# ebartrum/lightning_gan_zoo

Hardware: AMD Instinct MI355X
Metric: images/sec (G+D step) at 64x64 bs=128/GPU (higher is better)
Workload: dtype f32; 1 GPU; dc_gan synthetic 64x64 bs=128/GPU, one optimizer cycle of 2 batches (Lightning alternation + toggle), reference optimizer, fp32; key=dc_gan_bs128, global_batch=128, parallelism=dp1, images_counted=2*bs*n_gpus per step (every batch of the cycle)

## Files before the change

include/gz_ops.h:

```cpp
#ifndef GZ_OPS_H
#define GZ_OPS_H

#include <stddef.h>

#ifdef __cplusplus
extern "C" {
#endif

#ifndef __HIP__
typedef struct ihipStream_t* hipStream_t;
#endif

#define GZ_ACT_NONE 0
#define GZ_ACT_RELU 1
#define GZ_ACT_LRELU 2
#define GZ_ACT_TANH 3


long long gz_conv2d_pack_fwd_elems(int K, int C, int KH, int KW);
long long gz_conv2d_pack_dgrad_elems(int K, int C, int KH, int KW, int S);

int gz_conv2d_pack_fwd(const float* w, float* wpack, int K, int C, int KH, int KW, hipStream_t stream);
int gz_conv2d_pack_dgrad(const float* w, float* wpack, int K, int C, int KH, int KW, int S, int P,
                         hipStream_t stream);
// ... 104 lines not shown
                      int PH, int PW, int act, float slope, hipStream_t stream);
int gz_conv2d_fwd_any_into(const float* x, const float* wpack, const float* bias, float* y, int y_image_channels, int N,
                           int C, int H, int W, int K, int OH, int OW, int KH, int KW, int SH, int SW, int PH, int PW,
                           int act, float slope, hipStream_t stream);
int gz_pool2d(const float* x, float* y, long long planes, int H, int W, int OH, int OW, int KS, int S, int P, int mode,
              hipStream_t stream);
int gz_resize_bilinear(const float* x, float* y, long long planes, int H, int W, int OH, int OW, float mul, float add,
                       hipStream_t stream);

int gz_bce_logits_mean(const float* x, float* loss, int n, float target, hipStream_t stream);
int gz_bce_logits_mean_bwd(const float* x, const float* gloss, float* dx, int n, float target, hipStream_t stream);
int gz_pair_loss(const float* x, float* loss, int n_each, float t0, float t1, int mode, hipStream_t stream);
int gz_pair_loss_bwd(const float* x, const float* gloss, float* dx, int n_each, float t0, float t1, int mode,
                     hipStream_t stream);
int gz_gp_penalty(const float* sumsq, float* out, int n, hipStream_t stream);
int gz_gp_penalty_bwd(const float* sumsq, const float* gout, float* dsumsq, int n, hipStream_t stream);
int gz_mse_mean(const float* a, const float* b, float* loss, int n, hipStream_t stream);
int gz_mse_mean_bwd(const float* a, const float* b, const float* gloss, float* da, int n, hipStream_t stream);
int gz_vec_normalize(const float* x, float* out, float* out2, float* norm_out, int n, float eps, hipStream_t stream);
int gz_vec_normalize_dot(const float* x, float* out, float* out2, float* dot_out, int n, float eps,
                         hipStream_t stream);
int gz_vec_dot(const float* a, const float* b, float* out, int n, hipStream_t stream);
int gz_sn_max_jobs(void);
size_t gz_sn_table_bytes(void);
long long gz_sn_workspace_floats(int R, int L);
int gz_sn_add(void* table_host, const float* W, float* u, float* v, float* us, float* vs, float* sigma, float* workspace,
              int R, int L);
int gz_sn_power_iteration(void* table_host, float eps, hipStream_t stream);
int gz_sn_sigma_coef_floats(int groups);
int gz_sn_sigma_term(const float* rowsums, const float* rstd, const float* sigma, const float* u, const float* v,
                     float* coefs, float* term, int rows, int groups, int R, int L, float eps, hipStream_t stream);
int gz_div_scalar(const float* x, const float* sigma, float* out, long long count, hipStream_t stream);
int gz_spectral_norm_bwd(const float* g, const float* rowdots, const float* u, const float* v, const float* sigma,
                         float* out, int R, int L, hipStream_t stream);

size_t gz_norm_workspace_bytes(int N, int C);
int gz_norm_coef_elems(int N, int C, int per_channel);

int gz_batchnorm_finalize(const float* partials, int rows, long long count, const float* gamma, const float* beta,
                          float* coef, float* running_mean, float* running_var, long long* num_batches_tracked, int C,
                          float eps, float momentum, hipStream_t stream);
int gz_batchnorm_stats(const float* x, const float* gamma, const float* beta, float* coef, float* running_mean,
                       float* running_var, long long* num_batches_tracked, void* workspace, int N, int C,
                       int inner, float eps, float momentum, hipStream_t stream);
int gz_channel_sum(const float* x, float* out, void* workspace, int N, int C, int inner, hipStream_t stream);
int gz_batchnorm_eval_coef(const float* gamma, const float* beta, const float* running_mean,
                           const float* running_var, float* coef, int C, float eps, hipStream_t stream);
int gz_rownorm_stats(const float* x, const float* gamma, const float* beta, float* coef, void* workspace, int N,
                     int C, int inner, float eps, int affine_per_row, int unbiased, hipStream_t stream);
int gz_rownorm_act_fwd(const float* x, const float* gamma, const float* beta, float* coef, float* out, int N, int C,
                       int inner, float eps, int affine_per_row, int unbiased, int act, float slope,
                       hipStream_t stream);
int gz_adain_const_fwd(const float* x, const float* sb, float* coef, float* out, int N, int C, int inner, float eps,
                       int act, float slope, hipStream_t stream);
int gz_adain_const_bwd(const float* gout, const float* x, const float* coef, float* dx, float* dsb, int N, int C,
                       int inner, int act, float slope, hipStream_t stream);
int gz_norm_act_fwd(const float* x, const float* coef, float* out, int N, int C, int inner, int per_channel,
                    int act, float slope, hipStream_t stream);
int gz_rownorm_act_fwd_sigma(const float* x, const float* sigma, int groups, float* coef, float* out, int N, int C,
                             int inner, float eps, int act, float slope, hipStream_t stream);
int gz_rownorm_act_bwd_rows(const float* gout, const float* x, const float* coef, float* dx, float* rowsums, int N, int C,
                            int inner, int act, float slope, hipStream_t stream);
int gz_norm_act_bwd(const float* gout, const float* x, const float* coef, float* dx, float* dgamma, float* dbeta,
                    void* workspace, float* kbuf, int N, int C, int inner, int per_channel, int affine_per_row,
                    int unbiased, int act, float slope, hipStream_t stream);
int gz_batchnorm_stats_g(const float* x, const float* gamma, const float* beta, float* coef, float* running_mean,
                         float* running_var, long long* num_batches_tracked, void* workspace, int N, int C,
                         int inner, float eps, float momentum, int groups, hipStream_t stream);
int gz_batchnorm_finalize_g(const float* partials, int rows, long long count, const float* gamma, const float* beta,
                            float* coef, float* running_mean, float* running_var, long long* num_batches_tracked,
                            int C, float eps, float momentum, int groups, hipStream_t stream);
int gz_batchnorm_act_fwd_fused(const float* x, const float* partials, int rows, long long count, const float* gamma,
                               const float* beta, float* coef, float* running_mean, float* running_var,
                               long long* num_batches_tracked, void* workspace, float* out, int N, int C, int inner,
                               float eps, float momentum, int groups, int act, float slope, hipStream_t stream);
int gz_norm_act_fwd_g(const float* x, const float* coef, float* out, int N, int C, int inner, int per_channel,
                      int groups, int act, float slope, hipStream_t stream);
int gz_rownorm_act_bwd_acc(const float* gout, const float* x, const float* coef, float* dx, float* dgamma, float* dbeta,
                           void* workspace, float* kbuf, int N, int C, int inner, int act, float slope, int accumulate,
                           hipStream_t stream);
int gz_batchnorm_act_bwd_g(const float* gout, const float* x, const float* coef, float* dx, float* dgamma, float* dbeta,
                           void* workspace, float* kbuf, int N, int C, int inner, int act, float slope, int groups,
                           int accumulate, hipStream_t stream);

int gz_rownorm_act_bwd2(const float* gout, const float* v, const float* x, const float* coef, float* gg_out,
                        float* gx, float* ggamma, void* workspace, int N, int C, int inner, int act, float slope,
                        hipStream_t stream);
int gz_act_bwd(const float* g, const float* out, float* dx, long long count, int act, float slope,
               hipStream_t stream);
int gz_tanh_bwd2(const float* v, const float* g, const float* out, float* res, long long count, hipStream_t stream);

int gz_rowdot(const float* a, const float* b, float* y, int R, int L, int b_broadcast, hipStream_t stream);
int gz_rowscale(const float* x, const float* s, const float* x2, const float* s2, float* out, int R, int L,
                int x_broadcast, int one_minus_s, hipStream_t stream);
int gz_linear_multi_max_jobs(void);
size_t gz_linear_multi_table_bytes(void);
int gz_linear_multi_add(void* table_host, const float* weight, const float* bias, float* out, const float* g, float* dw,
                        float* db, int J);
int gz_linear_multi_fwd(void* table_host, const float* x, int N, int K, int act, float slope, hipStream_t stream);
int gz_linear_multi_bwd(void* table_host, const float* x, int N, int K, int act, float slope, hipStream_t stream);
int gz_colsum(const float* x, float* out, int R, int L, hipStream_t stream);
size_t gz_coldot_workspace_bytes(int R, int L);
int gz_coldot(const float* g, const float* x, float* out, float* workspace, size_t ws_bytes, int R, int L,
              hipStream_t stream);
int gz_coldot_partial(const float* g, const float* x, float* out, float* workspace, size_t ws_bytes, int R, int L,
                      int* nz_out, hipStream_t stream);
int gz_copy_words(const void* src, void* dst, long long words, hipStream_t stream);
int gz_clamp_(float* p, long long count, float lo, float hi, hipStream_t stream);

int gz_act_fwd(const float* x, float* y, long long count, int act, float slope, hipStream_t stream);
int gz_axpby(const float* a, float alpha, const float* b, float beta, float* out, float* act_out, long long count,
             int act, float slope, hipStream_t stream);
int gz_avgpool3s2_fwd(const float* x, float* y, long long planes, int H, int W, int OH, int OW, hipStream_t stream);
int gz_avgpool3s2_bwd(const float* gy, float* gx, long long planes, int H, int W, int OH, int OW,
                      hipStream_t stream);
int gz_upsample2_fwd(const float* x, float* y, long long planes, int H, int W, hipStream_t stream);
int gz_upsample2_bwd(const float* gy, float* gx, long long planes, int H, int W, hipStream_t stream);

int gz_u8hwc_to_nchw(const unsigned char* in, float* out, int N, int H, int W, int C, float mean, float std,
                     hipStream_t stream);

#define GZ_OPT_MAX_TENSORS 24
int gz_adam_step(int count, float* const* params, float* const* grads, float* const* exp_avg,
                 float* const* exp_avg_sq, const long long* numel, float lr, float beta1, float beta2, float eps,
                 int step, float grad_scale, int zero_grads, hipStream_t stream);
int gz_adam_src_max_tensors(void);
size_t gz_adam_src_table_bytes(void);
int gz_adam_src_add(void* table_host, float* param, float* exp_avg, float* exp_avg_sq, long long numel,
                    const float* slabs, int nz, long long stride);
int gz_adam_step_from_slabs(void* table_host, float lr, float beta1, float beta2, float eps, int step, float grad_scale,
                            hipStream_t stream);
int gz_adam_tick(float* tick, float beta1, float beta2, hipStream_t stream);
int gz_adam_step_dev(int count, float* const* params, float* const* grads, float* const* exp_avg,
                     float* const* exp_avg_sq, const long long* numel, float lr, float beta1, float beta2, float eps,
                     const float* tick, float grad_scale, int zero_grads, hipStream_t stream);
int gz_rmsprop_step(int count, float* const* params, float* const* grads, float* const* square_avg,
                    const long long* numel, float lr, float alpha, float eps, float grad_scale, int zero_grads,
                    hipStream_t stream);

const char* gz_last_error(void);

const char* gz_build_info(void);
const char* gz_source_digest(void);

#ifdef __cplusplus
}
#endif
#endif
```

lightning_gan_zoo_amd/csrc/gz_knobs.h:

```cpp
#pragma once
#include <stdlib.h>
#include <string.h>
#include <atomic>

namespace gz {

#define GZ_KNOB_LIST(X)                                                                                               \
                                                                                          \
    X(bool, no_igemm2, "GZ_NO_IGEMM2", false)                        \
    X(bool, no_igemm2_tap, "GZ_NO_IGEMM2_TAP", false)                      \
    X(bool, no_plane_a, "GZ_NO_PLANE_A", false)                \
    X(bool, no_wg3r, "GZ_NO_WG3R", false)                               \
    X(int, wg3r_wgs, "GZ_WG3R_WGS", 2)                              \
    X(int, wg3r_min_chunks, "GZ_WG3R_MIN_CHUNKS", 24)                         \
    X(bool, no_fewk_wg, "GZ_NO_FEWK_WG", false)               \
    X(bool, no_fewk_conv, "GZ_NO_FEWK_CONV", false)            \
    X(int, dg3_tile, "GZ_DG3_TILE", 0)                       \
    X(int, dg3_wgs, "GZ_DG3_WGS", 2)                         \
    X(int, dg3_min_chunks, "GZ_DG3_MIN_CHUNKS", 32)                            \
    X(bool, no_igemm2_wg, "GZ_NO_IGEMM2_WG", false)                              \
    X(bool, no_igemm2w, "GZ_NO_IGEMM2W", false)              \
    X(bool, no_igemm2wg, "GZ_NO_IGEMM2WG", false)                          \
    X(int, igemm2_tile, "GZ_IGEMM2_TILE", 0)                                 \
    X(bool, no_tile64, "GZ_NO_TILE64", false)                                  \
    X(bool, no_kg2, "GZ_NO_KG2", false)                             \
    X(bool, no_pool_plane, "GZ_NO_POOL_PLANE", false)               \
    X(bool, no_pool_group, "GZ_NO_POOL_GROUP", false)                  \
    X(bool, no_any2, "GZ_NO_ANY2", false)                    \
    X(bool, no_dg5, "GZ_NO_DG5", false)                      \
    X(int, dg5_wgs, "GZ_DG5_WGS", 512)                              \
    X(int, dg5_min_chunks, "GZ_DG5_MIN_CHUNKS", 24)             \
    X(int, dg5_min_units, "GZ_DG5_MIN_UNITS", 80)             \
    X(int, kg2_min_chunks, "GZ_KG2_MIN_CHUNKS", 32)                           \
    X(int, tap64_min_chunks, "GZ_TAP64_MIN_CHUNKS", 32)      \
    X(int, tile, "GZ_TILE", -1)                                               \
    X(int, min_wgs, "GZ_MIN_WGS", 0)                                \
    X(bool, no_big_split, "GZ_NO_BIG_SPLIT", false)                                                                   \
    X(bool, no_splitk, "GZ_NO_SPLITK", false)                                                                         \
    X(int, split_target, "GZ_SPLIT_TARGET", 1024)                                                                     \
    X(int, split_below, "GZ_SPLIT_BELOW", 512)                                                                        \
    X(bool, no_tapmajor, "GZ_NO_TAPMAJOR", false)                                                                     \
    X(bool, no_row4, "GZ_NO_ROW4", false)                                                                             \
    X(int, fwd2_min_tiles, "GZ_FWD2_MIN_TILES", 16)                                                                   \
    X(int, dg2_min_tiles, "GZ_DG2_MIN_TILES", 64)                                                                     \
    X(int, tap_wgs, "GZ_TAP_WGS", 384)                                                                                \
    X(int, tap_cps_max, "GZ_TAP_CPS_MAX", 96)                                                                         \
    X(int, wg_target, "GZ_WG_TARGET", 1024)                                                                           \
    X(int, wg2_min_chunks, "GZ_WG2_MIN_CHUNKS", 0)                                                                    \
    X(bool, wg_generic, "GZ_WG_GENERIC", false)                                                                       \
                                                                                                  \
    X(bool, no_smallc, "GZ_NO_SMALLC", false)                                                                         \
    X(bool, no_smallc5, "GZ_NO_SMALLC5", false)                                                                       \
    X(bool, smallc_one_pos, "GZ_SMALLC_ONE_POS", false)                                                               \
    X(long long, smallc_split_below, "GZ_SMALLC_SPLIT_BELOW", 192 * 1024)                                             \
    X(long long, smallc_split8_below, "GZ_SMALLC_SPLIT8_BELOW", 36 * 1024)                                            \
    X(int, smallc_ks, "GZ_SMALLC_KS", 0)                                                                              \
    X(bool, no_fewc_wg, "GZ_NO_FEWC_WG", false)                                                                       \
    X(bool, no_act_fuse, "GZ_NO_ACT_FUSE", false)                                                                     \
    X(bool, no_pack_k4, "GZ_NO_PACK_K4", false)                                                                       \
    X(bool, no_resample_swizzle, "GZ_NO_RESAMPLE_SWIZZLE", false)                                                     \
    X(int, fewc_wg_blocks, "GZ_FEWC_WG_BLOCKS", 512)                                                                  \
    X(bool, no_smallch_conv, "GZ_NO_SMALLCH_CONV", false)                                                             \
    X(bool, no_smallch_wg, "GZ_NO_SMALLCH_WG", false)                                                                 \
    X(int, c3_gpw, "GZ_C3_GPW", 4)                                                                                    \
                                                                                        \
    X(bool, no_xcd_swizzle, "GZ_NO_XCD_SWIZZLE", false)                                                               \
    X(int, dyn_lds, "GZ_DYN_LDS", 0)                                                                                  \
    X(int, igemm2_stagger, "GZ_IGEMM2_STAGGER", 0)                                                                    \
    X(int, igemm2_lds, "GZ_IGEMM2_LDS", 0)                                                                            \
                                                                     \
    X(bool, dg3_even_split, "GZ_DG3_EVEN_SPLIT", false)                                                               \
    X(int, wg3_target, "GZ_WG3_TARGET", 1024)                                                                         \
    X(int, wg3_tile, "GZ_WG3_TILE", -1)                                                                               \
    X(bool, norm_unfused, "GZ_NORM_UNFUSED", false)                                                                   \
    X(int, norm_bwd_cache, "GZ_NORM_BWD_CACHE", 4)                                                                    \
    X(bool, resample_fwd_direct, "GZ_RESAMPLE_FWD_DIRECT", false)                                                     \
    X(int, resample_bwd_mode, "GZ_RESAMPLE_BWD", 0)

struct Knobs {
    bool experiments;
#define GZ_KNOB_FIELD(type, name, env, dflt) type name;
    GZ_KNOB_LIST(GZ_KNOB_FIELD)
#undef GZ_KNOB_FIELD
};

inline void knob_read(bool& v, const char* e) { v = e != nullptr; }
inline void knob_read(int& v, const char* e) {
    if (!e) return;
    if (!strcmp(e, "scatter")) v = 1;
    else if (!strcmp(e, "gather")) v = 2;
    else v = atoi(e);
}
inline void knob_read(long long& v, const char* e) { if (e) v = atoll(e); }

inline const Knobs& knobs() {
    static const Knobs k = [] {
        Knobs n;
#define GZ_KNOB_INIT(type, name, env, dflt) n.name = dflt;
        GZ_KNOB_LIST(GZ_KNOB_INIT)
#undef GZ_KNOB_INIT
        const char* on = getenv("GZ_EXPERIMENTS");
        n.experiments = on && on[0] && on[0] != '0';
        if (n.experiments) {
#define GZ_KNOB_ENV(type, name, env, dflt) knob_read(n.name, getenv(env));
            GZ_KNOB_LIST(GZ_KNOB_ENV)
#undef GZ_KNOB_ENV
        }
        return n;
    }();
    return k;
}

inline std::atomic<int>& cu_budget_ref() {
    static std::atomic<int> v{256};
    return v;
}
inline int cus() { return cu_budget_ref().load(std::memory_order_relaxed); }

}
```

lightning_gan_zoo_amd/csrc/gz_norm.hip:

```cpp
#include "gz_common.h"
#include "gz_knobs.h"
#include "../../include/gz_ops.h"

namespace gz {

constexpr int PW_THREADS = 256;

struct RowGeom {
    int rows, q4;
    int lpr, rpw;
};

static RowGeom row_geom(long long rows, int inner) {
    RowGeom g;
    g.rows = (int)rows;
    g.q4 = inner / 4;
    int lpr = 1;
    while (lpr < 64 && lpr < g.q4) lpr <<= 1;
    g.lpr = lpr;
    g.rpw = 64 / lpr;
    return g;
}

static int row_grid(const RowGeom& g) {
    long long groups = ((long long)g.rows + g.rpw - 1) / g.rpw;
    long long blocks = (groups + 3) / 4;
    if (blocks > 256 * 8) blocks = 256 * 8;
    if (blocks < 1) blocks = 1;
    return (int)blocks;
}

template <int NS>
__device__ __forceinline__ void sub_reduce(float (&s)[NS], int lpr) {
    for (int o = lpr >> 1; o > 0; o >>= 1) {
#pragma unroll
        for (int k = 0; k < NS; ++k) s[k] += __shfl_xor(s[k], o, 64);
    }
}

__global__ __launch_bounds__(PW_THREADS) void row_sums_kernel(const float* __restrict__ x, f32x2* __restrict__ sums,
                                                              RowGeom g) {
    const int lane = threadIdx.x & 63;
    const int wave = (blockIdx.x * PW_THREADS + threadIdx.x) >> 6;
    const int nwaves = (gridDim.x * PW_THREADS) >> 6;
    const int sub = lane / g.lpr, l = lane % g.lpr;
    for (long long row0 = (long long)wave * g.rpw; row0 < g.rows; row0 += (long long)nwaves * g.rpw) {
        long long row = row0 + sub;
        float s[2] = {0.f, 0.f};
        if (row < g.rows) {
            const f32x4* p = reinterpret_cast<const f32x4*>(x) + row * g.q4;
            for (int q = l; q < g.q4; q += g.lpr) {
                f32x4 v = p[q];
                s[0] += (v.x + v.y) + (v.z + v.w);
                s[1] += (v.x * v.x + v.y * v.y) + (v.z * v.z + v.w * v.w);
            }
        }
        sub_reduce<2>(s, g.lpr);
        if (row < g.rows && l == 0) sums[row] = f32x2{s[0], s[1]};
    }
}

__global__ __launch_bounds__(64) void channel_sum_finalize_kernel(const f32x2* __restrict__ sums, float* __restrict__ out,
                                                                  int N, int C) {
    const int c = blockIdx.x, lane = threadIdx.x;
    double s = 0.0;
    for (int n = lane; n < N; n += 64) s += (double)sums[(long long)n * C + c].x;
    s = wave_sum_d(s);
    if (lane == 0) out[c] = (float)s;
}

template <int WAVES>
__global__ __launch_bounds__(64 * WAVES) void bn_finalize_kernel(const f32x2* __restrict__ sums,
                                                         const float* __restrict__ gamma,
                                                         const float* __restrict__ beta, float* __restrict__ coef,
                                                         float* running_mean, float* running_var, long long* nbt,
                                                         int N, int C, int inner, float eps, float momentum,
                                                         double count, int groups) {
    const int c = blockIdx.x, lane = threadIdx.x;
    if (c == 0 && lane == 0 && nbt) *nbt += groups;
    const int Ng = N / groups, NC = groups * C;
    for (int g = 0; g < groups; ++g) {
        double s1 = 0.0, s2 = 0.0;
// ... 32 lines not shown
        coef[NC + ci] = be - (float)mean * scale;
        coef[2 * NC + ci] = (float)mean;
        coef[3 * NC + ci] = rstd;
        if (running_mean) {
            double unbiased = cnt > 1.0 ? var * cnt / (cnt - 1.0) : var;
            running_mean[c] = (1.f - momentum) * running_mean[c] + momentum * (float)mean;
            running_var[c] = (1.f - momentum) * running_var[c] + momentum * (float)unbiased;
        }
    }
}

__global__ void bn_eval_coef_kernel(const float* __restrict__ gamma, const float* __restrict__ beta,
                                    const float* __restrict__ rm, const float* __restrict__ rv,
                                    float* __restrict__ coef, int C, float eps) {
    int c = blockIdx.x * blockDim.x + threadIdx.x;
    if (c >= C) return;
    float rstd = 1.f / sqrtf(rv[c] + eps);
    float ga = gamma ? gamma[c] : 1.f, be = beta ? beta[c] : 0.f;
    coef[c] = ga * rstd;
    coef[C + c] = be - rm[c] * ga * rstd;
    coef[2 * C + c] = rm[c];
    coef[3 * C + c] = rstd;
}

struct ApplyGeom {
    long long total4;
    int q4;
    FastDiv div_q4, div_c;
    int C, per_channel, ncoef;
    int group_rows;
    FastDiv div_grows;
};

__device__ __forceinline__ int coef_index(long long i4, const ApplyGeom& g) {
    uint32_t row = fdiv((uint32_t)i4, g.div_q4);
    if (g.per_channel) {
        const uint32_t grp = g.group_rows ? fdiv(row, g.div_grows) : 0u;
        row = row - fdiv(row, g.div_c) * (uint32_t)g.C + grp * (uint32_t)g.C;
    }
    return (int)row;
}

__global__ __launch_bounds__(PW_THREADS) void norm_act_apply_kernel(const float* __restrict__ x,
                                                                    const float* __restrict__ coef,
                                                                    float* __restrict__ out, ApplyGeom g, int act,
                                                                    float slope) {
    const long long stride = (long long)gridDim.x * PW_THREADS;
    for (long long i = (long long)blockIdx.x * PW_THREADS + threadIdx.x; i < g.total4; i += stride) {
        int ci = coef_index(i, g);
        float sc = coef[ci], sh = coef[g.ncoef + ci];
        f32x4 v = reinterpret_cast<const f32x4*>(x)[i];
        f32x4 o;
#pragma unroll
        for (int k = 0; k < 4; ++k) o[k] = act_fwd(v[k] * sc + sh, act, slope);
        reinterpret_cast<f32x4*>(out)[i] = o;
    }
}

struct BnFuse {
    int N, C, q4, groups, Ng, S, P;
    int CB, run4;
    FastDiv div_q4, div_run;
};

static BnFuse bn_fuse_geom(int N, int C, int inner, int groups) {
    BnFuse f;
    f.N = N; f.C = C; f.q4 = inner / 4; f.groups = groups; f.Ng = N / groups;
    int cb = 1;
    while (cb < 16 && cb * f.q4 < 64 && C % (cb * 2) == 0) cb *= 2;
    f.CB = cb;
    f.run4 = cb * f.q4;
    f.div_q4 = make_fastdiv(f.q4);
    f.div_run = make_fastdiv(f.run4);
    const long long per_cg = (long long)f.Ng * f.run4;
    const long long blocks = (long long)(C / cb) * groups;
    int S = 1;
    while (blocks * S < 1024 && S * 2 <= f.Ng && per_cg / (S * 2) >= 512) S *= 2;
    f.S = S;
    f.P = (f.Ng + S - 1) / S;
    return f;
}

__device__ __forceinline__ void block_channel_sums(const f32x2* __restrict__ base, long long stride, int count, int CB,
                                                   double (*red)[2]) {
    const int tid = threadIdx.x, cb = tid % CB, rr = tid / CB, lanes = PW_THREADS / CB;
    double s1 = 0.0, s2 = 0.0;
    for (int r = rr; r < count; r += lanes) {
        const f32x2 v = base[(long long)r * stride + cb];
        s1 += (double)v.x;
        s2 += (double)v.y;
    }
    __syncthreads();
    red[tid][0] = s1;
    red[tid][1] = s2;
    __syncthreads();
    for (int h = lanes >> 1; h >= 1; h >>= 1) {
        if (rr < h) {
            red[tid][0] += red[tid + h * CB][0];
            red[tid][1] += red[tid + h * CB][1];
        }
        __syncthreads();
    }
}

__global__ __launch_bounds__(PW_THREADS) void bn_apply_fused_kernel(
    const float* __restrict__ x, const f32x2* __restrict__ sums, int rows, double count, const float* __restrict__ gamma,
    const float* __restrict__ beta, float* __restrict__ coef, float* running_mean, float* running_var, long long* nbt,
    float* __restrict__ out, BnFuse f, int inner, float eps, float momentum, int act, float slope) {
    __shared__ double red[PW_THREADS][2];
    __shared__ float mine[16][2];
    const int tid = threadIdx.x;
    const int s = blockIdx.x % f.S, bg = blockIdx.x / f.S, g = bg % f.groups, c0 = (bg / f.groups) * f.CB;
    const bool owner = g == 0 && s == 0;
    const int Rg = rows / f.groups, NC = f.groups * f.C;
    for (int gg = 0; gg < f.groups; ++gg) {
        if (!owner && gg != g) continue;
        block_channel_sums(sums + (long long)gg * Rg * f.C + c0, f.C, Rg, f.CB, red);
        if (tid < f.CB) {
            const int c = c0 + tid;
            const double s1 = red[tid][0], s2 = red[tid][1];
            const double cnt = count > 0.0 ? count : (double)f.Ng * inner;
            const double mean = s1 / cnt;
            double var = s2 / cnt - mean * mean;
            if (var < 0.0) var = 0.0;
            const float rstd = (float)(1.0 / sqrt(var + (double)eps));
            const float ga = gamma ? gamma[c] : 1.f, be = beta ? beta[c] : 0.f;
            const float scale = ga * rstd, shift = be - (float)mean * scale;
            if (gg == g) {
                mine[tid][0] = scale;
                mine[tid][1] = shift;
            }
            if (owner) {
                const int ci = gg * f.C + c;
                coef[ci] = scale;
                coef[NC + ci] = shift;
                coef[2 * NC + ci] = (float)mean;
                coef[3 * NC + ci] = rstd;
                if (running_mean) {
                    const double unbiased = cnt > 1.0 ? var * cnt / (cnt - 1.0) : var;
                    running_mean[c] = (1.f - momentum) * running_mean[c] + momentum * (float)mean;
                    running_var[c] = (1.f - momentum) * running_var[c] + momentum * (float)unbiased;
                }
            }
        }
    }
    if (owner && c0 == 0 && tid == 0 && nbt) *nbt += f.groups;
    __syncthreads();
    const int n0 = g * f.Ng + s * f.P;
    const int n1 = min(g * f.Ng + f.Ng, n0 + f.P);
    const int total = (n1 - n0) * f.run4;
    const f32x4* __restrict__ x4 = reinterpret_cast<const f32x4*>(x);
    f32x4* __restrict__ o4 = reinterpret_cast<f32x4*>(out);
    for (int i = tid; i < total; i += PW_THREADS) {
        const uint32_t p = fdiv((uint32_t)i, f.div_run);
        const uint32_t rem = (uint32_t)i - p * (uint32_t)f.run4;
        const uint32_t cb = fdiv(rem, f.div_q4);
        const long long idx = ((long long)(n0 + (int)p) * f.C + c0) * f.q4 + rem;
        const float sc = mine[cb][0], sh = mine[cb][1];
        const f32x4 v = x4[idx];
        f32x4 o;
#pragma unroll
        for (int k = 0; k < 4; ++k) o[k] = act_fwd(v[k] * sc + sh, act, slope);
        o4[idx] = o;
    }
}

template <int CACHE>
__global__ __launch_bounds__(PW_THREADS) void rownorm_act_fused_kernel(const float* __restrict__ x,
                                                                       const float* __restrict__ gamma,
                                                                       const float* __restrict__ beta,
                                                                       float* __restrict__ coef,
                                                                       float* __restrict__ out, RowGeom g, int C,
                                                                       int inner, float eps, int affine_per_row,
                                                                       int unbiased, int act, float slope,
                                                                       int x_rows, const float* __restrict__ sigma,
                                                                       int sigma_rows) {
    const int lane = threadIdx.x & 63;
// ... 19 lines not shown
                s[0] += (v.x + v.y) + (v.z + v.w);
            }
        }
        sub_reduce<1>(s, g.lpr);
        const double cnt = (double)inner;
        const float mean_f = (float)((double)s[0] / cnt);
        float d[2] = {0.f, 0.f};
        if constexpr (CACHE > 0) {
#pragma unroll
            for (int i = 0; i < CACHE; ++i) {
                if (live && l + i * g.lpr < g.q4) {
#pragma unroll
                    for (int k = 0; k < 4; ++k) {
                        const float e = c[i][k] - mean_f;
                        d[0] += e;
                        d[1] += e * e;
                    }
                }
            }
        } else if (live) {
            for (int q = l; q < g.q4; q += g.lpr) {
                f32x4 v = p[q];
#pragma unroll
                for (int k = 0; k < 4; ++k) {
                    const float e = v[k] - mean_f;
                    d[0] += e;
                    d[1] += e * e;
                }
            }
        }
        sub_reduce<2>(d, g.lpr);
        if (!live) continue;
        const int r = (int)row;
        const double mean = (double)mean_f + (double)d[0] / cnt;
        double var = ((double)d[1] - (double)d[0] * (double)d[0] / cnt) / cnt;
        if (var < 0.0) var = 0.0;
        if (unbiased && inner > 1) var = var * cnt / (cnt - 1.0);
        float eps_r = eps;
        if (sigma) {
            const float sg = sigma[r / sigma_rows];
            eps_r = eps * sg * sg;
        }
        const float rstd = (float)(1.0 / sqrt(var + (double)eps_r));
        const int gi = affine_per_row == 2 ? (r / C) * 2 * C + r % C : (affine_per_row ? r : r % C);
        const float ga = gamma ? gamma[gi] : 1.f, be = beta ? beta[gi] : 0.f;
        const float sc = ga * rstd;
        const float sh = be - (float)mean * sc;
        if (l == 0) {
            coef[r] = sc;
            coef[g.rows + r] = sh;
            coef[2 * g.rows + r] = (float)mean;
            coef[3 * g.rows + r] = rstd;
        }
        if (!out) continue;
        f32x4* po = reinterpret_cast<f32x4*>(out) + row * g.q4;
        if constexpr (CACHE > 0) {
#pragma unroll
            for (int i = 0; i < CACHE; ++i) {
                const int q = l + i * g.lpr;
                if (q < g.q4) {
                    f32x4 o;
#pragma unroll
                    for (int k = 0; k < 4; ++k) o[k] = act_fwd(c[i][k] * sc + sh, act, slope);
                    po[q] = o;
                }
            }
        } else {
            for (int q = l; q < g.q4; q += g.lpr) {
                f32x4 v = p[q], o;
#pragma unroll
                for (int k = 0; k < 4; ++k) o[k] = act_fwd(v[k] * sc + sh, act, slope);
                po[q] = o;
            }
        }
    }
}

__device__ __forceinline__ float act_grad_z(float z, int act, float slope) {
    if (act == ACT_RELU) return z > 0.f ? 1.f : 0.f;
    if (act == ACT_LRELU) return z > 0.f ? 1.f : slope;
    return 1.f;
}

__global__ __launch_bounds__(PW_THREADS) void norm_bwd_rowsums_kernel(const float* __restrict__ gout,
                                                                      const float* __restrict__ x,
                                                                      const float* __restrict__ coef,
                                                                      f32x2* __restrict__ sums, RowGeom g, int C,
                                                                      int per_channel, int ncoef, int act,
                                                                      float slope, int group_rows) {
    const int lane = threadIdx.x & 63;
    const int wave = (blockIdx.x * PW_THREADS + threadIdx.x) >> 6;
    const int nwaves = (gridDim.x * PW_THREADS) >> 6;
    const int sub = lane / g.lpr, l = lane % g.lpr;
    for (long long row0 = (long long)wave * g.rpw; row0 < g.rows; row0 += (long long)nwaves * g.rpw) {
        long long row = row0 + sub;
        float s[2] = {0.f, 0.f};
        if (row < g.rows) {
            int ci = per_channel ? (int)(row % C) + (group_rows ? (int)(row / group_rows) * C : 0) : (int)row;
            float sc = coef[ci], sh = coef[ncoef + ci], mean = coef[2 * ncoef + ci], rstd = coef[3 * ncoef + ci];
            const f32x4* px = reinterpret_cast<const f32x4*>(x) + row * g.q4;
            const f32x4* pg = reinterpret_cast<const f32x4*>(gout) + row * g.q4;
            for (int q = l; q < g.q4; q += g.lpr) {
                f32x4 xv = px[q], gv = pg[q];
#pragma unroll
                for (int k = 0; k < 4; ++k) {
                    float dz = gv[k] * act_grad_z(xv[k] * sc + sh, act, slope);
                    s[0] += dz;
                    s[1] += dz * ((xv[k] - mean) * rstd);
                }
            }
        }
        sub_reduce<2>(s, g.lpr);
        if (row < g.rows && l == 0) sums[row] = f32x2{s[0], s[1]};
    }
}

__global__ __launch_bounds__(64) void bn_bwd_finalize_kernel(const f32x2* __restrict__ sums, float* __restrict__ k,
                                                             float* __restrict__ dgamma, float* __restrict__ dbeta,
                                                             int N, int C, int inner, int groups, int accumulate) {
    const int c = blockIdx.x, lane = threadIdx.x;
    const int Ng = N / groups, NC = groups * C;
    double t1 = 0.0, t2 = 0.0;
    for (int g = 0; g < groups; ++g) {
        double s1 = 0.0, s2 = 0.0;
        for (int n = lane; n < Ng; n += 64) {
            f32x2 v = sums[(long long)(g * Ng + n) * C + c];
            s1 += (double)v.x;
            s2 += (double)v.y;
        }
        s1 = wave_sum_d(s1);
        s2 = wave_sum_d(s2);
        if (lane == 0) {
            double cnt = (double)Ng * inner;
            k[g * C + c] = (float)(s1 / cnt);
            k[NC + g * C + c] = (float)(s2 / cnt);
        }
        t1 += s1;
        t2 += s2;
    }
    if (lane != 0) return;
    if (dgamma) dgamma[c] = (accumulate ? dgamma[c] : 0.f) + (float)t2;
    if (dbeta) dbeta[c] = (accumulate ? dbeta[c] : 0.f) + (float)t1;
}

__global__ void row_bwd_finalize_kernel(const f32x2* __restrict__ sums, float* __restrict__ k,
                                        float* __restrict__ dgamma, float* __restrict__ dbeta, int N, int C,
                                        int inner, int affine_per_row, int unbiased) {
    int i = blockIdx.x * blockDim.x + threadIdx.x;
    int rows = N * C;
    if (i < rows) {
        f32x2 v = sums[i];
        k[i] = v.x / (float)inner;
        k[rows + i] = v.y / (float)((unbiased && inner > 1) ? inner - 1 : inner);
        if (affine_per_row) {
            const int gi = affine_per_row == 2 ? (i / C) * 2 * C + i % C : i;
            if (dgamma) dgamma[gi] = v.y;
            if (dbeta) dbeta[gi] = v.x;
        }
    }
}

__global__ __launch_bounds__(64) void row_bwd_affine_kernel(const f32x2* __restrict__ sums,
                                                            float* __restrict__ dgamma, float* __restrict__ dbeta,
                                                            int N, int C, int accumulate = 0) {
    const int c = blockIdx.x, lane = threadIdx.x;
    double s1 = 0.0, s2 = 0.0;
    for (int n = lane; n < N; n += 64) {
        f32x2 v = sums[(long long)n * C + c];
        s1 += (double)v.x;
        s2 += (double)v.y;
    }
    s1 = wave_sum_d(s1);
    s2 = wave_sum_d(s2);
    if (lane != 0) return;
    if (dgamma) dgamma[c] = (accumulate ? dgamma[c] : 0.f) + (float)s2;
    if (dbeta) dbeta[c] = (accumulate ? dbeta[c] : 0.f) + (float)s1;
}

__global__ __launch_bounds__(PW_THREADS) void norm_bwd_apply_kernel(const float* __restrict__ gout,
                                                                    const float* __restrict__ x,
                                                                    const float* __restrict__ coef,
                                                                    const float* __restrict__ k,
                                                                    float* __restrict__ dx, ApplyGeom g, int act,
                                                                    float slope) {
    const long long stride = (long long)gridDim.x * PW_THREADS;
    for (long long i = (long long)blockIdx.x * PW_THREADS + threadIdx.x; i < g.total4; i += stride) {
        int ci = coef_index(i, g);
        float sc = coef[ci], sh = coef[g.ncoef + ci], mean = coef[2 * g.ncoef + ci], rstd = coef[3 * g.ncoef + ci];
        float k1 = k[ci], k2 = k[g.ncoef + ci];
        f32x4 xv = reinterpret_cast<const f32x4*>(x)[i];
        f32x4 gv = reinterpret_cast<const f32x4*>(gout)[i];
        f32x4 o;
#pragma unroll
        for (int q = 0; q < 4; ++q) {
            float dz = gv[q] * act_grad_z(xv[q] * sc + sh, act, slope);
            float xh = (xv[q] - mean) * rstd;
            o[q] = sc * (dz - k1 - xh * k2);
        }
        reinterpret_cast<f32x4*>(dx)[i] = o;
    }
}

__global__ __launch_bounds__(PW_THREADS) void bn_bwd_apply_fused_kernel(
    const float* __restrict__ gout, const float* __restrict__ x, const float* __restrict__ coef,
    const f32x2* __restrict__ sums, float* __restrict__ kout, float* __restrict__ dgamma, float* __restrict__ dbeta,
    float* __restrict__ dx, BnFuse f, int inner, int act, float slope, int accumulate) {
    __shared__ double red[PW_THREADS][2];
    __shared__ float mine[16][6];
    const int tid = threadIdx.x;
    const int s = blockIdx.x % f.S, bg = blockIdx.x / f.S, g = bg % f.groups, c0 = (bg / f.groups) * f.CB;
    const bool owner = g == 0 && s == 0;
    const int NC = f.groups * f.C;
    double t1 = 0.0, t2 = 0.0;
    for (int gg = 0; gg < f.groups; ++gg) {
        if (!owner && gg != g) continue;
        block_channel_sums(sums + (long long)gg * f.Ng * f.C + c0, f.C, f.Ng, f.CB, red);
        if (tid < f.CB) {
            const double s1 = red[tid][0], s2 = red[tid][1];
            const double cnt = (double)f.Ng * inner;
            const float k1 = (float)(s1 / cnt), k2 = (float)(s2 / cnt);
            if (gg == g) {
                mine[tid][0] = k1;
                mine[tid][1] = k2;
            }
            if (owner && kout) {
                kout[gg * f.C + c0 + tid] = k1;
                kout[NC + gg * f.C + c0 + tid] = k2;
            }
            t1 += s1;
            t2 += s2;
        }
    }
    if (tid < f.CB) {
        const int c = c0 + tid, ci = g * f.C + c;
        if (owner) {
            if (dgamma) dgamma[c] = (accumulate ? dgamma[c] : 0.f) + (float)t2;
            if (dbeta) dbeta[c] = (accumulate ? dbeta[c] : 0.f) + (float)t1;
        }
        mine[tid][2] = coef[ci];
        mine[tid][3] = coef[NC + ci];
        mine[tid][4] = coef[2 * NC + ci];
        mine[tid][5] = coef[3 * NC + ci];
    }
    __syncthreads();
    const int n0 = g * f.Ng + s * f.P;
    const int n1 = min(g * f.Ng + f.Ng, n0 + f.P);
    const int total = (n1 - n0) * f.run4;
    const f32x4* __restrict__ x4 = reinterpret_cast<const f32x4*>(x);
    const f32x4* __restrict__ g4 = reinterpret_cast<const f32x4*>(gout);
    f32x4* __restrict__ d4 = reinterpret_cast<f32x4*>(dx);
    for (int i = tid; i < total; i += PW_THREADS) {
        const uint32_t p = fdiv((uint32_t)i, f.div_run);
        const uint32_t rem = (uint32_t)i - p * (uint32_t)f.run4;
        const uint32_t cb = fdiv(rem, f.div_q4);
        const long long idx = ((long long)(n0 + (int)p) * f.C + c0) * f.q4 + rem;
        const float k1 = mine[cb][0], k2 = mine[cb][1], sc = mine[cb][2], sh = mine[cb][3], mean = mine[cb][4],
                    rstd = mine[cb][5];
        const f32x4 xv = x4[idx], gv = g4[idx];
        f32x4 o;
#pragma unroll
        for (int q = 0; q < 4; ++q) {
            const float dz = gv[q] * act_grad_z(xv[q] * sc + sh, act, slope);
            const float xh = (xv[q] - mean) * rstd;
            o[q] = sc * (dz - k1 - xh * k2);
        }
        d4[idx] = o;
    }
}

template <int CACHE>
__global__ __launch_bounds__(PW_THREADS) void rownorm_bwd_fused_kernel(const float* __restrict__ gout,
                                                                       const float* __restrict__ x,
                                                                       const float* __restrict__ coef,
                                                                       float* __restrict__ dx,
                                                                       float* __restrict__ dgamma,
                                                                       float* __restrict__ dbeta,
                                                                       f32x2* __restrict__ sums, RowGeom g, int C,
                                                                       int inner, int affine_per_row, int unbiased,
                                                                       int act, float slope) {
    const int lane = threadIdx.x & 63;
    const int wave = (blockIdx.x * PW_THREADS + threadIdx.x) >> 6;
    const int nwaves = (gridDim.x * PW_THREADS) >> 6;
    const int sub = lane / g.lpr, l = lane % g.lpr;
    for (long long row0 = (long long)wave * g.rpw; row0 < g.rows; row0 += (long long)nwaves * g.rpw) {
        const long long row = row0 + sub;
        const bool live = row < g.rows;
        const int ci = live ? (int)row : 0;
        const float sc = coef[ci], sh = coef[g.rows + ci], mean = coef[2 * g.rows + ci], rstd = coef[3 * g.rows + ci];
        const f32x4* px = reinterpret_cast<const f32x4*>(x) + row * g.q4;
        const f32x4* pg = reinterpret_cast<const f32x4*>(gout) + row * g.q4;
        float s[2] = {0.f, 0.f};
        f32x4 cdz[CACHE > 0 ? CACHE : 1], cxh[CACHE > 0 ? CACHE : 1];
        if constexpr (CACHE > 0) {
#pragma unroll
            for (int i = 0; i < CACHE; ++i) {
                const int q = l + i * g.lpr;
                const bool in = live && q < g.q4;
                const f32x4 xv = in ? px[q] : f32x4{0.f, 0.f, 0.f, 0.f};
                const f32x4 gv = in ? pg[q] : f32x4{0.f, 0.f, 0.f, 0.f};
#pragma unroll
                for (int k = 0; k < 4; ++k) {
                    const float dz = gv[k] * act_grad_z(xv[k] * sc + sh, act, slope);
                    const float xh = (xv[k] - mean) * rstd;
                    cdz[i][k] = dz;
                    cxh[i][k] = xh;
                    s[0] += dz;
                    s[1] += dz * xh;
                }
            }
        } else if (live) {
            for (int q = l; q < g.q4; q += g.lpr) {
                f32x4 xv = px[q], gv = pg[q];
#pragma unroll
                for (int k = 0; k < 4; ++k) {
                    float dz = gv[k] * act_grad_z(xv[k] * sc + sh, act, slope);
                    s[0] += dz;
                    s[1] += dz * ((xv[k] - mean) * rstd);
                }
            }
        }
        sub_reduce<2>(s, g.lpr);
        if (!live) continue;
        const float k1 = s[0] / (float)inner;
        const float k2 = s[1] / (float)((unbiased && inner > 1) ? inner - 1 : inner);
        if (l == 0) {
            if (sums) sums[row] = f32x2{s[0], s[1]};
            if (affine_per_row) {
                const int r = (int)row;
                const int gi = affine_per_row == 2 ? (r / C) * 2 * C + r % C : r;
                if (dgamma) dgamma[gi] = s[1];
                if (dbeta) dbeta[gi] = s[0];
            }
        }
        if (!dx) continue;
        f32x4* po = reinterpret_cast<f32x4*>(dx) + row * g.q4;
        if constexpr (CACHE > 0) {
#pragma unroll
            for (int i = 0; i < CACHE; ++i) {
                const int q = l + i * g.lpr;
                if (q < g.q4) {
                    f32x4 o;
#pragma unroll
                    for (int k = 0; k < 4; ++k) o[k] = sc * (cdz[i][k] - k1 - cxh[i][k] * k2);
                    po[q] = o;
                }
            }
        } else {
            for (int q = l; q < g.q4; q += g.lpr) {
                f32x4 xv = px[q], gv = pg[q], o;
#pragma unroll
// ... 354 lines not shown
                         (N / groups) * C);
    return launch_status();
}

int gz_rownorm_act_bwd_rows(const float* gout, const float* x, const float* coef, float* dx, float* rowsums, int N, int C,
                            int inner, int act, float slope, hipStream_t stream) {
    gz::clear_stale_error();
    if (!norm_shape_ok(N, C, inner) || !dx || !rowsums) return GZ_ERR_BAD_SHAPE;
    RowGeom rg = row_geom((long long)N * C, inner);
    const int per_lane = (rg.q4 + rg.lpr - 1) / rg.lpr;
    const int max_cache = knobs().norm_bwd_cache;
#define GZ_RB(CACHE)                                                                                                  \
    hipLaunchKernelGGL(rownorm_bwd_fused_kernel<CACHE>, dim3(row_grid(rg)), dim3(PW_THREADS), 0, stream, gout, x, coef, \
                       dx, (float*)nullptr, (float*)nullptr, (f32x2*)rowsums, rg, C, inner, 0, 0, act, slope)
    if (per_lane <= 1) GZ_RB(1);
    else if (per_lane <= 4 && max_cache >= 4) GZ_RB(4);
    else if (per_lane <= 16 && max_cache >= 16) GZ_RB(16);
    else GZ_RB(0);
#undef GZ_RB
    return launch_status();
}

int gz_adain_const_fwd(const float* x, const float* sb, float* coef, float* out, int N, int C, int inner, float eps,
                       int act, float slope, hipStream_t stream) {
    gz::clear_stale_error();
    if (!norm_shape_ok(N, C, inner)) return GZ_ERR_BAD_SHAPE;
    RowGeom g = row_geom((long long)N * C, inner);
    launch_rownorm_fused(x, sb, sb + C, coef, out, g, C, inner, eps, 2, 1, act, slope, stream, C);
    return launch_status();
}

int gz_adain_const_bwd(const float* gout, const float* x, const float* coef, float* dx, float* dsb, int N, int C,
                       int inner, int act, float slope, hipStream_t stream) {
    gz::clear_stale_error();
    if (!norm_shape_ok(N, C, inner)) return GZ_ERR_BAD_SHAPE;
    RowGeom g = row_geom(C, inner);
    if ((g.q4 + g.lpr - 1) / g.lpr > 4) return GZ_ERR_UNSUPPORTED;
    hipLaunchKernelGGL(adain_const_bwd_kernel, dim3(C), dim3(PW_THREADS), 0, stream, gout, x, coef, dx, dsb, g, N, C,
                       inner, act, slope);
    return launch_status();
}

int gz_norm_act_fwd_g(const float* x, const float* coef, float* out, int N, int C, int inner, int per_channel,
                      int groups, int act, float slope, hipStream_t stream) {
    gz::clear_stale_error();
    if (!norm_shape_ok(N, C, inner) || !groups_ok(N, groups) || (groups > 1 && !per_channel)) return GZ_ERR_BAD_SHAPE;
    ApplyGeom g = apply_geom(N, C, inner, per_channel, groups);
    hipLaunchKernelGGL(norm_act_apply_kernel, dim3(ew_grid(g.total4)), dim3(PW_THREADS), 0, stream, x, coef, out, g,
                       act, slope);
    return launch_status();
}

int gz_norm_act_fwd(const float* x, const float* coef, float* out, int N, int C, int inner, int per_channel,
                    int act, float slope, hipStream_t stream) {
    return gz_norm_act_fwd_g(x, coef, out, N, C, inner, per_channel, 1, act, slope, stream);
}

static int norm_act_bwd_impl(const float* gout, const float* x, const float* coef, float* dx, float* dgamma, float* dbeta,
                             void* workspace, float* kbuf, int N, int C, int inner, int per_channel, int affine_per_row,
                             int unbiased, int act, float slope, int groups, int accumulate, hipStream_t stream);

int gz_norm_act_bwd(const float* gout, const float* x, const float* coef, float* dx, float* dgamma, float* dbeta,
                    void* workspace, float* kbuf, int N, int C, int inner, int per_channel, int affine_per_row,
                    int unbiased, int act, float slope, hipStream_t stream) {
    return norm_act_bwd_impl(gout, x, coef, dx, dgamma, dbeta, workspace, kbuf, N, C, inner, per_channel, affine_per_row,
                             unbiased, act, slope, 1, 0, stream);
}

int gz_rownorm_act_bwd_acc(const float* gout, const float* x, const float* coef, float* dx, float* dgamma, float* dbeta,
                           void* workspace, float* kbuf, int N, int C, int inner, int act, float slope, int accumulate,
                           hipStream_t stream) {
    return norm_act_bwd_impl(gout, x, coef, dx, dgamma, dbeta, workspace, kbuf, N, C, inner, 0, 0, 0, act, slope, 1,
                             accumulate, stream);
}

int gz_batchnorm_act_bwd_g(const float* gout, const float* x, const float* coef, float* dx, float* dgamma, float* dbeta,
                           void* workspace, float* kbuf, int N, int C, int inner, int act, float slope, int groups,
                           int accumulate, hipStream_t stream) {
    if (!groups_ok(N, groups)) return GZ_ERR_BAD_SHAPE;
    return norm_act_bwd_impl(gout, x, coef, dx, dgamma, dbeta, workspace, kbuf, N, C, inner, 1, 0, 0, act, slope, groups,
                             accumulate, stream);
}

static int norm_act_bwd_impl(const float* gout, const float* x, const float* coef, float* dx, float* dgamma, float* dbeta,
                             void* workspace, float* kbuf, int N, int C, int inner, int per_channel, int affine_per_row,
                             int unbiased, int act, float slope, int groups, int accumulate, hipStream_t stream) {
    gz::clear_stale_error();
    if (!norm_shape_ok(N, C, inner)) return GZ_ERR_BAD_SHAPE;
    RowGeom rg = row_geom((long long)N * C, inner);
    ApplyGeom g = apply_geom(N, C, inner, per_channel, groups);
    const bool unfused = knobs().norm_unfused;
    if (!per_channel && !unfused) {
        const bool channel_affine = !affine_per_row && (dgamma || dbeta);
        const int max_cache = knobs().norm_bwd_cache;
        const int per_lane = (rg.q4 + rg.lpr - 1) / rg.lpr;
#define GZ_RB(CACHE)                                                                                                  \
    hipLaunchKernelGGL(rownorm_bwd_fused_kernel<CACHE>, dim3(row_grid(rg)), dim3(PW_THREADS), 0, stream, gout, x, coef, \
                       dx, dgamma, dbeta, channel_affine ? (f32x2*)workspace : (f32x2*)nullptr, rg, C, inner,          \
                       affine_per_row, unbiased, act, slope)
        if (per_lane <= 1) GZ_RB(1);
        else if (per_lane <= 4 && max_cache >= 4) GZ_RB(4);
        else if (per_lane <= 16 && max_cache >= 16) GZ_RB(16);
        else GZ_RB(0);
#undef GZ_RB
        if (channel_affine)
            hipLaunchKernelGGL(row_bwd_affine_kernel, dim3(C), dim3(64), 0, stream, (const f32x2*)workspace, dgamma,
                               dbeta, N, C, accumulate);
        return launch_status();
    }
    hipLaunchKernelGGL(norm_bwd_rowsums_kernel, dim3(row_grid(rg)), dim3(PW_THREADS), 0, stream, gout, x, coef,
                       (f32x2*)workspace, rg, C, per_channel, g.ncoef, act, slope, g.group_rows);
    if (per_channel && dx && !unfused) {
        const BnFuse f = bn_fuse_geom(N, C, inner, groups);
        hipLaunchKernelGGL(bn_bwd_apply_fused_kernel, dim3((C / f.CB) * groups * f.S), dim3(PW_THREADS), 0, stream, gout, x, coef,
                           (const f32x2*)workspace, kbuf, dgamma, dbeta, dx, f, inner, act, slope, accumulate);
        return launch_status();
    }
    if (per_channel) {
        hipLaunchKernelGGL(bn_bwd_finalize_kernel, dim3(C), dim3(64), 0, stream, (const f32x2*)workspace, kbuf, dgamma,
                           dbeta, N, C, inner, groups, accumulate);
    } else {
        int rows = N * C;
        hipLaunchKernelGGL(row_bwd_finalize_kernel, dim3((rows + 255) / 256), dim3(256), 0, stream,
                           (const f32x2*)workspace, kbuf, dgamma, dbeta, N, C, inner, affine_per_row, unbiased);
        if (!affine_per_row && (dgamma || dbeta))
            hipLaunchKernelGGL(row_bwd_affine_kernel, dim3(C), dim3(64), 0, stream, (const f32x2*)workspace, dgamma,
                               dbeta, N, C, accumulate);
    }
    if (dx)
        hipLaunchKernelGGL(norm_bwd_apply_kernel, dim3(ew_grid(g.total4)), dim3(PW_THREADS), 0, stream, gout, x, coef,
                           kbuf, dx, g, act, slope);
    return launch_status();
}

int gz_rownorm_act_bwd2(const float* gout, const float* v, const float* x, const float* coef, float* gg_out,
                        float* gx, float* ggamma, void* workspace, int N, int C, int inner, int act, float slope,
                        hipStream_t stream) {
    gz::clear_stale_error();
    if (!norm_shape_ok(N, C, inner)) return GZ_ERR_BAD_SHAPE;
    RowGeom rg = row_geom((long long)N * C, inner);
    ApplyGeom g = apply_geom(N, C, inner, 0);
    hipLaunchKernelGGL(norm_bwd2_rowsums_kernel, dim3(row_grid(rg)), dim3(PW_THREADS), 0, stream, gout, v, x, coef,
                       (Sums5*)workspace, rg, act, slope);
    if (gg_out || gx)
        hipLaunchKernelGGL(norm_bwd2_apply_kernel, dim3(ew_grid(g.total4)), dim3(PW_THREADS), 0, stream, gout, v, x,
                           coef, (const Sums5*)workspace, gg_out, gx, g, act, slope);
    if (ggamma)
        hipLaunchKernelGGL(norm_bwd2_ggamma_kernel, dim3(C), dim3(64), 0, stream, (const Sums5*)workspace, coef, ggamma,
                           N, C, inner);
    return launch_status();
}

int gz_act_bwd(const float* g, const float* out, float* dx, long long count, int act, float slope,
               hipStream_t stream) {
    gz::clear_stale_error();
    if (count <= 0 || (count & 3)) return GZ_ERR_BAD_SHAPE;
    hipLaunchKernelGGL(act_bwd_kernel, dim3(ew_grid(count / 4)), dim3(PW_THREADS), 0, stream, g, out, dx, count / 4,
                       act, slope);
    return launch_status();
}

int gz_tanh_bwd2(const float* v, const float* g, const float* out, float* res, long long count, hipStream_t stream) {
    gz::clear_stale_error();
    if (count <= 0 || (count & 3)) return GZ_ERR_BAD_SHAPE;
    hipLaunchKernelGGL(tanh_bwd2_kernel, dim3(ew_grid(count / 4)), dim3(PW_THREADS), 0, stream, v, g, out, res,
                       count / 4);
    return launch_status();
}

}
```

Baseline: 45010 images/s.

## Add single-launch register-resident batchnorm backward kernel for small spatial sizes

Result: no change. 45120 images/s (median of 6 runs) (+0.3%).

```diff
diff --git a/include/gz_ops.h b/include/gz_ops.h
--- a/include/gz_ops.h
+++ b/include/gz_ops.h
@@ -210,6 +210,7 @@
 int gz_batchnorm_act_bwd_g(const float* gout, const float* x, const float* coef, float* dx, float* dgamma, float* dbeta,
                            void* workspace, float* kbuf, int N, int C, int inner, int act, float slope, int groups,
                            int accumulate, hipStream_t stream);
+int gz_batchnorm_bwd_plan(int N, int C, int inner, int groups, char* buf, int buflen);
 
 int gz_rownorm_act_bwd2(const float* gout, const float* v, const float* x, const float* coef, float* gg_out,
                         float* gx, float* ggamma, void* workspace, int N, int C, int inner, int act, float slope,
diff --git a/lightning_gan_zoo_amd/csrc/gz_knobs.h b/lightning_gan_zoo_amd/csrc/gz_knobs.h
--- a/lightning_gan_zoo_amd/csrc/gz_knobs.h
+++ b/lightning_gan_zoo_amd/csrc/gz_knobs.h
@@ -74,6 +74,7 @@
     X(int, wg3_tile, "GZ_WG3_TILE", -1)                                                                               \
     X(bool, norm_unfused, "GZ_NORM_UNFUSED", false)                                                                   \
     X(int, norm_bwd_cache, "GZ_NORM_BWD_CACHE", 4)                                                                    \
+    X(int, bn_bwd_resident, "GZ_BN_BWD_RESIDENT", 1)              \
     X(bool, resample_fwd_direct, "GZ_RESAMPLE_FWD_DIRECT", false)                                                     \
     X(int, resample_bwd_mode, "GZ_RESAMPLE_BWD", 0)
 
diff --git a/lightning_gan_zoo_amd/csrc/gz_norm.hip b/lightning_gan_zoo_amd/csrc/gz_norm.hip
--- a/lightning_gan_zoo_amd/csrc/gz_norm.hip
+++ b/lightning_gan_zoo_amd/csrc/gz_norm.hip
@@ -1,3 +1,4 @@
+#include <stdio.h>
 #include "gz_common.h"
 #include "gz_knobs.h"
 #include "../../include/gz_ops.h"
@@ -196,17 +197,22 @@
 }
 
 __device__ __forceinline__ void block_channel_sums(const f32x2* __restrict__ base, long long stride, int count, int CB,
-                                                   double (*red)[2]) {
-    const int tid = threadIdx.x, cb = tid % CB, rr = tid / CB, lanes = PW_THREADS / CB;
+                                                   double (*red)[2], int lanes = 0) {
+    if (lanes == 0) lanes = PW_THREADS / CB;
+    const int tid = threadIdx.x, cb = tid % CB, rr = tid / CB;
+    const bool on = rr < lanes;
     double s1 = 0.0, s2 = 0.0;
-    for (int r = rr; r < count; r += lanes) {
-        const f32x2 v = base[(long long)r * stride + cb];
-        s1 += (double)v.x;
-        s2 += (double)v.y;
-    }
+    if (on)
+        for (int r = rr; r < count; r += lanes) {
+            const f32x2 v = base[(long long)r * stride + cb];
+            s1 += (double)v.x;
+            s2 += (double)v.y;
+        }
     __syncthreads();
-    red[tid][0] = s1;
-    red[tid][1] = s2;
+    if (on) {
+        red[tid][0] = s1;
+        red[tid][1] = s2;
+    }
     __syncthreads();
     for (int h = lanes >> 1; h >= 1; h >>= 1) {
         if (rr < h) {
@@ -392,6 +398,24 @@
     return 1.f;
 }
 
+__device__ __forceinline__ void bwd_elem(float xv, float gv, float sc, float sh, float mean, float rstd, int act,
+                                         float slope, float& a, float& dz, float& xh) {
+#pragma clang fp contract(off)
+    a = act_grad_z(__builtin_fmaf(xv, sc, sh), act, slope);
+    dz = gv * a;
+    xh = (xv - mean) * rstd;
+}
+__device__ __forceinline__ void bwd_row_acc(float (&s)[2], float dz, float xh) {
+#pragma clang fp contract(off)
+    s[0] += dz;
+    s[1] += dz * xh;
+}
+__device__ __forceinline__ float bwd_dx(float sc, float gv, float a, float xh, float k1, float k2, bool last) {
+#pragma clang fp contract(off)
+    const float t = last ? gv * a - k1 : __builtin_fmaf(gv, a, -k1);
+    return sc * __builtin_fmaf(-xh, k2, t);
+}
+
 __global__ __launch_bounds__(PW_THREADS) void norm_bwd_rowsums_kernel(const float* __restrict__ gout,
                                                                       const float* __restrict__ x,
                                                                       const float* __restrict__ coef,
@@ -414,9 +438,9 @@
                 f32x4 xv = px[q], gv = pg[q];
 #pragma unroll
                 for (int k = 0; k < 4; ++k) {
-                    float dz = gv[k] * act_grad_z(xv[k] * sc + sh, act, slope);
-                    s[0] += dz;
-                    s[1] += dz * ((xv[k] - mean) * rstd);
+                    float a, dz, xh;
+                    bwd_elem(xv[k], gv[k], sc, sh, mean, rstd, act, slope, a, dz, xh);
+                    bwd_row_acc(s, dz, xh);
                 }
             }
         }
@@ -570,12 +594,147 @@
         f32x4 o;
 #pragma unroll
         for (int q = 0; q < 4; ++q) {
-            const float dz = gv[q] * act_grad_z(xv[q] * sc + sh, act, slope);
-            const float xh = (xv[q] - mean) * rstd;
-            o[q] = sc * (dz - k1 - xh * k2);
+            float a, dz, xh;
+            bwd_elem(xv[q], gv[q], sc, sh, mean, rstd, act, slope, a, dz, xh);
+            o[q] = bwd_dx(sc, gv[q], a, xh, k1, k2, q == 3);
         }
         d4[idx] = o;
     }
+}
+
+constexpr int BN_RES_THREADS = 1024;
+constexpr int BN_RES_ITEMS = 8;
+constexpr int BN_RES_ROWS = 2048;
+
+struct BnRes {
+    int ok;
+    int N, C, q4, groups, Ng;
+    int lpr, lpr_sh;
+    int CBo, cbo_sh;
+    int lanes;
+    int T, items, dn;
+    FastDiv div_ng;
+};
+
+template <int ITEMS>
+__global__ __launch_bounds__(BN_RES_THREADS) void bn_bwd_resident_kernel(
+    const float* __restrict__ gout, const float* __restrict__ x, const float* __restrict__ coef,
+    float* __restrict__ kout, float* __restrict__ dgamma, float* __restrict__ dbeta, float* __restrict__ dx, BnRes r,
+    int inner, int act, float slope, int accumulate) {
+    __shared__ f32x2 rs[BN_RES_ROWS];
+    __shared__ double red[PW_THREADS][2];
+    __shared__ float kk[8][16][2];
+    __shared__ f32x4 cf[8][16];
+    const int tid = threadIdx.x, c0 = blockIdx.x * r.CBo;
+    const int l = tid & (r.lpr - 1), row0 = tid >> r.lpr_sh;
+    const int n0 = row0 >> r.cbo_sh, cb = row0 & (r.CBo - 1), c = c0 + cb;
+    const int NC = r.groups * r.C;
+    const bool in = l < r.q4;
+    const f32x4* __restrict__ x4 = reinterpret_cast<const f32x4*>(x);
+    const f32x4* __restrict__ g4 = reinterpret_cast<const f32x4*>(gout);
+    f32x4 cg[ITEMS], cx[ITEMS];
+#pragma unroll
+    for (int i = 0; i < ITEMS; ++i) {
+        const long long idx = ((long long)(n0 + i * r.dn) * r.C + c) * r.q4 + l;
+        cx[i] = in ? x4[idx] : f32x4{0.f, 0.f, 0.f, 0.f};
+        cg[i] = in ? g4[idx] : f32x4{0.f, 0.f, 0.f, 0.f};
+    }
+    if (tid < r.groups * r.CBo) {
+        const int ci = (tid >> r.cbo_sh) * r.C + c0 + (tid & (r.CBo - 1));
+        cf[tid >> r.cbo_sh][tid & (r.CBo - 1)] = f32x4{coef[ci], coef[NC + ci], coef[2 * NC + ci], coef[3 * NC + ci]};
+    }
+    __syncthreads();
+#pragma unroll
+    for (int i = 0; i < ITEMS; ++i) {
+        const int n = n0 + i * r.dn;
+        const f32x4 co = cf[fdiv((uint32_t)n, r.div_ng)][cb];
+        const float sc = co[0], sh = co[1], mean = co[2], rstd = co[3];
+        float s[2] = {0.f, 0.f};
+#pragma unroll
+        for (int k = 0; k < 4; ++k) {
+            float a, dz, xh;
+            bwd_elem(cx[i][k], cg[i][k], sc, sh, mean, rstd, act, slope, a, dz, xh);
+            bwd_row_acc(s, dz, xh);
+        }
+        sub_reduce<2>(s, r.lpr);
+        if (l == 0) rs[n * r.CBo + cb] = f32x2{s[0], s[1]};
+    }
+    __syncthreads();
+    double t1 = 0.0, t2 = 0.0;
+    for (int gg = 0; gg < r.groups; ++gg) {
+        block_channel_sums(rs + gg * r.Ng * r.CBo, r.CBo, r.Ng, r.CBo, red, r.lanes);
+        if (tid < r.CBo) {
+            const double s1 = red[tid][0], s2 = red[tid][1];
+            const double cnt = (double)r.Ng * inner;
+            const float k1 = (float)(s1 / cnt), k2 = (float)(s2 / cnt);
+            kk[gg][tid][0] = k1;
+            kk[gg][tid][1] = k2;
+            if (kout) {
+                kout[gg * r.C + c0 + tid] = k1;
+                kout[NC + gg * r.C + c0 + tid] = k2;
+            }
+            t1 += s1;
+            t2 += s2;
+        }
+    }
+    if (tid < r.CBo) {
+        const int c = c0 + tid;
+        if (dgamma) dgamma[c] = (accumulate ? dgamma[c] : 0.f) + (float)t2;
+        if (dbeta) dbeta[c] = (accumulate ? dbeta[c] : 0.f) + (float)t1;
+    }
+    __syncthreads();
+    if (!in) return;
+    f32x4* __restrict__ d4 = reinterpret_cast<f32x4*>(dx);
+#pragma unroll
+    for (int i = 0; i < ITEMS; ++i) {
+        const int n = n0 + i * r.dn;
+        const int gi = (int)fdiv((uint32_t)n, r.div_ng);
+        const f32x4 co = cf[gi][cb];
+        const float sc = co[0], sh = co[1], mean = co[2], rstd = co[3], k1 = kk[gi][cb][0], k2 = kk[gi][cb][1];
+        f32x4 o;
+#pragma unroll
+        for (int k = 0; k < 4; ++k) {
+            float a, dz, xh;
+            bwd_elem(cx[i][k], cg[i][k], sc, sh, mean, rstd, act, slope, a, dz, xh);
+            o[k] = bwd_dx(sc, cg[i][k], a, xh, k1, k2, k == 3);
+        }
+        d4[((long long)n * r.C + c) * r.q4 + l] = o;
+    }
+}
+
+static BnRes bn_res_geom(int N, int C, int inner, int groups) {
+    BnRes r{};
+    const BnFuse f = bn_fuse_geom(N, C, inner, groups);
+    if (f.q4 > 64 || groups > 8) return r;
+    const RowGeom rg = row_geom((long long)N * C, inner);
+    for (int cbo = f.CB; cbo >= 1; cbo >>= 1) {
+        const long long rows = (long long)N * cbo, slots = rows * rg.lpr;
+        if (rows > BN_RES_ROWS || slots > (long long)BN_RES_THREADS * BN_RES_ITEMS) continue;
+        int items = 0;
+        for (int it = BN_RES_ITEMS; it >= 1 && !items; it >>= 1)
+            if (N % it == 0 && slots % (it * 64) == 0 && slots / it >= PW_THREADS && slots / it <= BN_RES_THREADS)
+                items = it;
+        if (!items) continue;
+        r.ok = 1;
+        r.CBo = cbo;
+        r.items = items;
+        r.T = (int)(slots / items);
+        if (C / cbo >= 256) break;
+    }
+    if (!r.ok) return r;
+    r.N = N; r.C = C; r.q4 = f.q4; r.groups = groups; r.Ng = f.Ng;
+    r.lpr = rg.lpr;
+    r.lanes = PW_THREADS / f.CB;
+    r.dn = N / r.items;
+    for (r.lpr_sh = 0; (1 << r.lpr_sh) < r.lpr; ++r.lpr_sh) {}
+    for (r.cbo_sh = 0; (1 << r.cbo_sh) < r.CBo; ++r.cbo_sh) {}
+    r.div_ng = make_fastdiv(r.Ng);
+    return r;
+}
+
+static BnRes bn_bwd_choice(int N, int C, int inner, int groups) {
+    if (!knobs().bn_bwd_resident) return BnRes{};
+    return bn_res_geom(N, C, inner, groups);
 }
 
 template <int CACHE>
@@ -1096,6 +1255,20 @@
                              accumulate, stream);
 }
 
+int gz_batchnorm_bwd_plan(int N, int C, int inner, int groups, char* buf, int buflen) {
+    if (!buf || buflen <= 0) return GZ_ERR_BAD_SHAPE;
+    buf[0] = 0;
+    if (!norm_shape_ok(N, C, inner) || !groups_ok(N, groups)) return GZ_ERR_BAD_SHAPE;
+    if (knobs().norm_unfused) return snprintf(buf, (size_t)buflen, "unfused rowsums + finalize + apply");
+    const BnRes r = bn_bwd_choice(N, C, inner, groups);
+    if (r.ok)
+        return snprintf(buf, (size_t)buflen, "resident cb=%d wgs=%d threads=%d items=%d lanes=%d", r.CBo, C / r.CBo, r.T,
+                        r.items, r.lanes);
+    const BnFuse f = bn_fuse_geom(N, C, inner, groups);
+    return snprintf(buf, (size_t)buflen, "two-launch rowsums + apply cb=%d wgs=%d%s", f.CB, (C / f.CB) * groups * f.S,
+                    knobs().bn_bwd_resident ? "" : " (resident off)");
+}
+
 static int norm_act_bwd_impl(const float* gout, const float* x, const float* coef, float* dx, float* dgamma, float* dbeta,
                              void* workspace, float* kbuf, int N, int C, int inner, int per_channel, int affine_per_row,
                              int unbiased, int act, float slope, int groups, int accumulate, hipStream_t stream) {
@@ -1122,6 +1295,20 @@
                                dbeta, N, C, accumulate);
         return launch_status();
     }
+    if (per_channel && dx && !unfused) {
+        const BnRes r = bn_bwd_choice(N, C, inner, groups);
+        if (r.ok) {
+#define GZ_BR(ITEMS)                                                                                                  \
+    hipLaunchKernelGGL(bn_bwd_resident_kernel<ITEMS>, dim3(C / r.CBo), dim3(r.T), 0, stream, gout, x, coef, kbuf,     \
+                       dgamma, dbeta, dx, r, inner, act, slope, accumulate)
+            if (r.items == 8) GZ_BR(8);
+            else if (r.items == 4) GZ_BR(4);
+            else if (r.items == 2) GZ_BR(2);
+            else GZ_BR(1);
+#undef GZ_BR
+            return launch_status();
+        }
+    }
     hipLaunchKernelGGL(norm_bwd_rowsums_kernel, dim3(row_grid(rg)), dim3(PW_THREADS), 0, stream, gout, x, coef,
                        (f32x2*)workspace, rg, C, per_channel, g.ncoef, act, slope, g.group_rows);
     if (per_channel && dx && !unfused) {
```
